# ducha-aiki/affnet

Measured on AMD Instinct MI355X. Metric: keypoints/sec (detect+AffNet+OriNet+HardNet) per image, 2000 kp @1024x768, higher is better.
Workload: dtype f32

## Files before the change

### affnet_amd/_lib.py

```python
import ctypes as C
import os

_HERE = os.path.dirname(os.path.abspath(__file__))
LIB_PATH = os.environ.get("AFFNET_HIP_LIB") or os.path.join(_HERE, "libaffnet_hip.so")
PROBES_LIB_PATH = os.path.join(_HERE, "libaffnet_hip_probes.so")

MAX_OCTAVES, MAX_LEVELS, MAX_TAPS = 16, 8, 37
NET_AFFNET, NET_ORINET, NET_HARDNET, NET_AFFNET_FULLCONV = 0, 1, 2, 3
ARITH_FP32_MFMA, ARITH_FP32_SPLIT3, ARITH_FP32_SPLIT2H = 0, 1, 2
ARITH_NAMES = {"fp32": ARITH_FP32_MFMA, "fp32_mfma": ARITH_FP32_MFMA, "fp32_split3": ARITH_FP32_SPLIT3, "split3": ARITH_FP32_SPLIT3,
               "fp32_split2h": ARITH_FP32_SPLIT2H, "split2h": ARITH_FP32_SPLIT2H}


def arith_code(arith):
    if arith is None:
        return ARITH_FP32_MFMA
    if isinstance(arith, str):
        if arith.lower() not in ARITH_NAMES:
            raise ValueError("arith must be one of %s" % sorted(ARITH_NAMES))
        return ARITH_NAMES[arith.lower()]
    if int(arith) not in (ARITH_FP32_MFMA, ARITH_FP32_SPLIT3, ARITH_FP32_SPLIT2H):
        raise ValueError("arith must be AFFNET_ARITH_FP32_MFMA (0), AFFNET_ARITH_FP32_SPLIT3 (1) or AFFNET_ARITH_FP32_SPLIT2H (2)")
    return int(arith)
SHAPE_FORM_DIRECT, SHAPE_FORM_WINOGRAD = 0, 1
OK, ERR_INVALID, ERR_HIP, ERR_CAPACITY, ERR_EMPTY = 0, -1, -2, -3, -4


class Config(C.Structure):
    _fields_ = [
        ("height", C.c_int32), ("width", C.c_int32), ("n_octaves", C.c_int32), ("levels_per_octave", C.c_int32),
        ("oct_h", C.c_int32 * MAX_OCTAVES), ("oct_w", C.c_int32 * MAX_OCTAVES),
        ("level_sigma", (C.c_float * MAX_LEVELS) * MAX_OCTAVES),
        ("level_sigma4", (C.c_float * MAX_LEVELS) * MAX_OCTAVES),
        ("level_sigma_px", (C.c_double * MAX_LEVELS) * MAX_OCTAVES),
        ("first_blur_taps", C.c_int32), ("first_blur", C.c_float * (MAX_TAPS * MAX_TAPS)),
        ("level_blur_taps", C.c_int32 * MAX_LEVELS),
        ("level_blur", (C.c_float * (MAX_TAPS * MAX_TAPS)) * MAX_LEVELS),
        ("level_blur0_taps", C.c_int32 * MAX_LEVELS),
        ("level_blur0", (C.c_float * (MAX_TAPS * MAX_TAPS)) * MAX_LEVELS),
        ("lazy_shape_rows", C.c_int32),
        ("onepass", C.c_int32),
        ("mr_size", C.c_float), ("threshold", C.c_float),
        ("num_features", C.c_int32), ("num_prefilter", C.c_int32),
        ("max_raw_per_octave_div", C.c_int32), ("max_keep", C.c_int32), ("batch", C.c_int32), ("baum_iters", C.c_int32),
        ("arith", C.c_int32),
    ]


class Nets(C.Structure):
    _fields_ = [("d_affnet", C.c_void_p), ("d_orinet", C.c_void_p), ("d_hardnet", C.c_void_p),
                ("h_orientation_window", C.c_void_p), ("h_baumberg_window", C.c_void_p)]


_P, _I, _SZ = C.c_void_p, C.c_int, C.c_size_t
SYMBOLS = {
    "affnet_config_fill": (_I, [C.POINTER(Config), _I, _I, _I, C.c_double, _I, C.c_double, C.c_double, _I, _I, _I, _I]),
    "affnet_ctx_create": (_I, [C.POINTER(_P), _I, C.POINTER(Config)]),
    "affnet_ctx_destroy": (None, [_P]),
    "affnet_last_error": (C.c_char_p, [_P]),
    "affnet_version": (C.c_char_p, []),
    "affnet_set_arith": (_I, [_P, _I]),
    "affnet_get_arith": (_I, [_P]),
    "affnet_set_shape_form": (_I, [_P, _I]),
    "affnet_get_shape_form": (_I, [_P]),
    "affnet_workspace_bytes": (_SZ, [_P]),
    "affnet_bind_workspace": (_I, [_P, _P, _SZ]),
    "affnet_pyramid_level_offset": (C.c_int64, [_P, _I, _I]),
    "affnet_pyramid_image_stride": (C.c_int64, [_P]),
    "affnet_batch": (_I, [_P]),
    "affnet_capacity_prefilter": (_I, [_P]),
    "affnet_capacity_final": (_I, [_P]),
    "affnet_gauss_blur": (_I, [_P, _P, _P, _I, _I, C.POINTER(C.c_float), _I, _P]),
    "affnet_pyramid_build": (_I, [_P, _P, _P]),
    "affnet_hessian_response": (_I, [_P, _P, _P, _I, _I, C.c_float, _P]),
    "affnet_detect": (_I, [_P, _P, _P, _P, _P, _P]),
    "affnet_detect_responses": (_I, [_P, _P, _P, _P, _P, _P, _P]),
    "affnet_laf_grid_sample": (_I, [_P, _P, _I, _I, _P, _I, _I, _P, _P]),
    "affnet_pyr_grid_sample": (_I, [_P, _P, _P, _P, _I, _I, _P, _P]),
    "affnet_cnn32_packed_floats": (_SZ, [_I]),
    "affnet_cnn32_winograd_offset": (C.c_int64, [_I, _I]),
    "affnet_cnn32_pack_weights": (_I, [_I, C.POINTER(_P), C.POINTER(_P), C.POINTER(_P), _P, _P, _P, _P, _P]),
    "affnet_cnn32_forward": (_I, [_P, _I, _P, _P, _P, _I, _P, _P, _P]),
    "affnet_cnn32_forward_pyr": (_I, [_P, _I, _P, _P, _P, _P, _I, _P, _P, _P]),
    "affnet_local_norm": (_I, [_P, _P, _P, _I, _I, _P]),
    "affnet_fullconv_scratch_bytes": (_SZ, [_I, _I]),
    "affnet_fullconv_forward": (_I, [_P, _P, _P, _I, _I, _P, _P, _P]),
    "affnet_nms2d": (_I, [_P, _P, _P, _I, _I, C.c_float, _P]),
    "affnet_shape_filter_select": (_I, [_P, _P, _P, _P, _P, _P, _P, _P, _P, _P, _P]),
    "affnet_apply_rotation": (_I, [_P, _P, _P, _P, _I, _P]),
    "affnet_scale_lafs": (_I, [_P, _P, _P, _P, _I, _I, _I, _I, _P]),
    "affnet_lafs_to_ellipses": (_I, [_P, _P, _P, _I, _P, _P]),
    "affnet_ellipses_to_lafs": (_I, [_P, _P, _P, _I, _P, _P]),
    "affnet_level_select": (_I, [_P, _P, _P, _I, _I, _P, _P, _P]),
    "affnet_handcrafted_forward": (_I, [_P, _I, _P, _I, _P, _P, _P, _P]),
    "affnet_handcrafted_forward_pyr": (_I, [_P, _I, _P, _P, _P, _I, _P, _P, _P]),
    "affnet_sift_host_window": (_I, [_I, C.POINTER(C.c_float)]),
    "affnet_sift_forward": (_I, [_P, _P, _I, _P, C.c_float, _P, _P]),
    "affnet_sift_forward_pyr": (_I, [_P, _P, _P, _P, _I, _P, C.c_float, _P, _P]),
    "affnet_tfeat_packed_floats": (_SZ, []),
    "affnet_tfeat_pack_weights": (_I, [_P, _P, _P, _P, _P, _P, _P]),
    "affnet_tfeat_scratch_floats": (_SZ, [_I]),
    "affnet_tfeat_forward": (_I, [_P, _P, _P, _P, _I, _P, _P, _P]),
    "affnet_tfeat_forward_pyr": (_I, [_P, _P, _P, _P, _P, _I, _P, _P, _P]),
    "affnet_match_scratch_bytes": (_SZ, [_I, _I]),
    "affnet_distance_matrix": (_I, [_P, _P, _I, _P, _I, _I, _P, _P, _P]),
    "affnet_match_snn": (_I, [_P, _P, _I, _P, _I, _I, C.c_float, _P, _P, _P, _P, _P, _P, _P]),
    "affnet_reproject_lafs": (_I, [_P, _P, _I, C.POINTER(C.c_float), _P, _P]),
    "affnet_centre_nn": (_I, [_P, _P, _I, _P, _I, _P, _P, _P]),
    "affnet_extract_features": (_I, [_P, C.POINTER(Nets), _P, _I, _P, _P, _P, _P, _P, _P]),
    "affnet_detect_image": (_I, [_P, _P, _P]),
    "affnet_detect_image_responses": (_I, [_P, _P, _P]),
    "affnet_detect_image_onepass": (_I, [_P, _P, _P, _P]),
    "affnet_detect_image_onepass_responses": (_I, [_P, _P, _P, _P]),
    "affnet_detected_list": (_I, [_P, _P, _P, _P, _P, _P]),
    "affnet_load_frames": (_I, [_P, _P, _I, _P, _P, _P, _I, _I, _P]),
    "affnet_describe_frames": (_I, [_P, C.POINTER(Nets), _P, _P, _P, _P, _I, _I, _P, _P, _P, _P, _P, _P]),
    "affnet_shape_iterate": (_I, [_P, _P, _P, _P, _P, _I, _P, _P]),
    "affnet_affmap_offset": (C.c_int64, [_P, _I]),
    "affnet_affmap_image_stride": (C.c_int64, [_P]),
    "affnet_describe_detected": (_I, [_P, C.POINTER(Nets), _I, _P, _P, _P, _P, _P, _P]),
    "affnet_graph_capture_extract": (_I, [_P, C.POINTER(Nets), _P, _I, _P, _P, _P, _P, _P, _P]),
    "affnet_graph_launch": (_I, [_P, _P]),
    "affnet_profile_enable": (_I, [_P, _I]),
    "affnet_profile_read": (_I, [_P, C.POINTER(C.c_double * 8), C.POINTER(C.c_int32)]),
    "affnet_read_counts": (_I, [_P, C.POINTER(C.c_int32 * 4), _P]),
    "affnet_counter_offset": (C.c_int64, [_P, _I]),
    "affnet_counter_stride": (C.c_int64, [_P]),
    "affnet_host_base_grid": (_I, [_I, C.POINTER(C.c_float)]),
}

DEBUG_SYMBOLS = {
    "affnet_cnn32_debug_timing": (_I, [_P, _P]),
    "affnet_cnn32_debug_layer": (_I, [_P, _I, _P, _P, _I, _P, _P]),
    "affnet_cnn32_debug_winograd_u": (_I, [_P, _I, _P, _I, _P, _P]),
    "affnet_selftest_mfma": (_I, [_P, _P, _P, _P]),
    "affnet_debug_split3_variant": (_I, [_P, _I]),
}

PROBE_SYMBOLS = {
    "affnet_cnn32_probe": (_I, [_P, _I, _I, _I, _I, _P, _P]),
    "affnet_split3_gemm": (_I, [_P, _P, _I, _I, _I, _I, _P, _P]),
    "affnet_split3_rate": (_I, [_I, _I, _I, _P, _P]),
    "affnet_debug_stream": (_I, [_P, _P, _SZ, _I, _I, _I, _P]),
    "affnet_probe_shape_offsets": (_I, [_P, C.POINTER(C.c_int64 * 3)]),
}


class AffnetHipError(RuntimeError):
    pass


class AffnetEmptyError(AffnetHipError):
    """AFFNET_ERR_EMPTY: no image of the call produced a detection (the reference raises in torch.cat([]),
    SparseImgRepresenter.py:100)."""


def _load():
    if not os.path.isfile(LIB_PATH):
        if os.path.basename(LIB_PATH) == os.path.basename(PROBES_LIB_PATH):
            raise ImportError("affnet_amd: %s is missing - the tools under tools/ need the probe build of the library: "
                              "AFFNET_PROBES=1 bash affnet_amd/csrc/build.sh" % LIB_PATH)
        raise ImportError(
            "affnet_amd: %s is missing - the HIP extension is the only implementation of this path "
            "(no CPU fallback). Build it: bash affnet_amd/csrc/build.sh" % LIB_PATH)
    lib = C.CDLL(LIB_PATH)
    for table in (SYMBOLS, DEBUG_SYMBOLS):
        for name, (res, args) in table.items():
            fn = getattr(lib, name)
            fn.restype, fn.argtypes = res, args
    for name, (res, args) in PROBE_SYMBOLS.items():
        if hasattr(lib, name):
            fn = getattr(lib, name)
            fn.restype, fn.argtypes = res, args
    return lib


lib = _load()


def check(rc, ctx=None, what=""):
    if rc != OK:
        msg = lib.affnet_last_error(ctx).decode() if ctx else ""
        if rc == ERR_EMPTY:
            raise AffnetEmptyError("%s: %s" % (what or "libaffnet_hip call", msg))
        raise AffnetHipError("%s failed (code %d): %s" % (what or "libaffnet_hip call", rc, msg))


def ptr(t):
    return None if t is None else C.c_void_p(t.data_ptr())


def current_stream(device):
    import torch
    return C.c_void_p(torch.cuda.current_stream(device).cuda_stream)
```

### affnet_amd/csrc/cnn_trunk.h

```cpp
#pragma once
#include <math.h>

#include <type_traits>

#include "common.h"

#include "cnn_mfma.h"

template <int TM>
__device__ __forceinline__ void head_partials(const float* __restrict__ hw, const f32x4 (&bias)[1], const f32x4 (&acc)[TM][1],
                                              float* __restrict__ part, int wave, int lane) {
    constexpr int MT = 4, MG = MT / TM;
    const int mg = wave % MG, ng = wave / MG;
    const int n = lane & 15, g = lane >> 4;
    const int c4 = ng * 16 + 4 * g;
    f32x4 v[TM];
#pragma unroll
    for (int i = 0; i < TM; ++i) {
        v[i] = acc[i][0] + bias[0];
        v[i].x = fmaxf(v[i].x, 0.0f); v[i].y = fmaxf(v[i].y, 0.0f); v[i].z = fmaxf(v[i].z, 0.0f); v[i].w = fmaxf(v[i].w, 0.0f);
    }
    const __amdgpu_buffer_rsrc_t r = weight_rsrc(hw, 3 * 4096);
    f32x4 w[3][TM];
#pragma unroll
    for (int o = 0; o < 3; ++o)
#pragma unroll
        for (int i = 0; i < TM; ++i) w[o][i] = buf_read4(r, (n * 64 + c4) * 4, (o * 4096 + (mg * TM + i) * 16 * 64) * 4);
#pragma unroll
    for (int o = 0; o < 3; ++o) {
        float sacc = 0.f;
#pragma unroll
        for (int i = 0; i < TM; ++i)
#pragma unroll
            for (int j = 0; j < 4; ++j) sacc = fmaf(v[i][j], w[o][i][j], sacc);
        sacc = wave_sum(sacc);
        if (lane == 0) part[wave * 4 + o] = sacc;
    }
}

#define ORI_HP 68
struct OriHeadLane {
    int mg, n, c4;
    template <int TM>
    __device__ __forceinline__ static OriHeadLane of(int wave, int lane) {
        constexpr int MT = 4, MG = MT / TM;
        const int mg = wave % MG, ng = wave / MG;
        const int n = lane & 15, g = lane >> 4;
        return {mg, n, ng * 16 + 4 * g};
    }
};
template <int TM>
__device__ __forceinline__ void ori_head_weights(const float* __restrict__ hw, const OriHeadLane& L, f32x4 (&w)[2][TM]) {
    const __amdgpu_buffer_rsrc_t r = weight_rsrc(hw, 2 * 4096);
#pragma unroll
    for (int o = 0; o < 2; ++o)
#pragma unroll
        for (int i = 0; i < TM; ++i) w[o][i] = buf_read4(r, (L.n * 64 + L.c4) * 4, (o * 4096 + (L.mg * TM + i) * 16 * 64) * 4);
}
template <int NTHR>
__device__ __forceinline__ void ori_head_zero_halo(float* act, int tid) {
    for (int e = tid; e < 36 * 16; e += NTHR) {
        const int hp = e >> 4, q4 = e & 15;
        const int y = hp < 10 ? 0 : (hp < 20 ? 9 : 1 + ((hp - 20) >> 1)), x = hp < 10 ? hp : (hp < 20 ? hp - 10 : ((hp - 20) & 1) * 9);
        *reinterpret_cast<f32x4*>(&act[(y * 10 + x) * ORI_HP + 4 * q4]) = (f32x4){0.f, 0.f, 0.f, 0.f};
    }
}
template <int TM>
__device__ __forceinline__ void ori_head_pbase(const OriHeadLane& L, int (&pbase)[TM]) {
#pragma unroll
    for (int i = 0; i < TM; ++i) {
        const int p = (L.mg * TM + i) * 16 + L.n;
        pbase[i] = ((p >> 3) * 10 + (p & 7)) * ORI_HP + L.c4;
    }
}
template <int TM>
__device__ __forceinline__ void ori_head_reduce(const f32x4 (&w)[2][TM], const int (&pbase)[TM], float* __restrict__ part, const float* act, int wave, int lane) {
    __syncthreads();
#pragma unroll
    for (int q = 0; q < 9; ++q) {
        float s0 = 0.f, s1 = 0.f;
#pragma unroll
        for (int i = 0; i < TM; ++i) {
            const f32x4 av = *reinterpret_cast<const f32x4*>(&act[pbase[i] + ((q / 3) * 10 + q % 3) * ORI_HP]);
#pragma unroll
            for (int j = 0; j < 4; ++j) { s0 = fmaf(av[j], w[0][i][j], s0); s1 = fmaf(av[j], w[1][i][j], s1); }
        }
        s0 = wave_sum(s0);
        s1 = wave_sum(s1);
        if (lane == 0) { part[wave * 18 + q] = s0; part[wave * 18 + 9 + q] = s1; }
    }
}
template <int TM, int NTHR>
__device__ __forceinline__ void head_partials_ori_lds(const float* __restrict__ hw, const f32x4 (&bias)[1], const f32x4 (&acc)[TM][1],
                                                      float* __restrict__ part, float* act, int wave, int lane, int tid) {
    constexpr int MT = 4, MG = MT / TM;
    const int mg = wave % MG, ng = wave / MG;
    const int n = lane & 15, g = lane >> 4;
    const int c4 = ng * 16 + 4 * g;
    f32x4 v[TM];
#pragma unroll
    for (int i = 0; i < TM; ++i) {
        v[i] = acc[i][0] + bias[0];
        v[i].x = fmaxf(v[i].x, 0.0f); v[i].y = fmaxf(v[i].y, 0.0f); v[i].z = fmaxf(v[i].z, 0.0f); v[i].w = fmaxf(v[i].w, 0.0f);
    }
    const __amdgpu_buffer_rsrc_t r = weight_rsrc(hw, 2 * 4096);
    f32x4 w[2][TM];
#pragma unroll
    for (int o = 0; o < 2; ++o)
#pragma unroll
        for (int i = 0; i < TM; ++i) w[o][i] = buf_read4(r, (n * 64 + c4) * 4, (o * 4096 + (mg * TM + i) * 16 * 64) * 4);
    __syncthreads();
    for (int e = tid; e < 36 * 16; e += NTHR) {
        const int hp = e >> 4, q4 = e & 15;
        const int y = hp < 10 ? 0 : (hp < 20 ? 9 : 1 + ((hp - 20) >> 1)), x = hp < 10 ? hp : (hp < 20 ? hp - 10 : ((hp - 20) & 1) * 9);
        *reinterpret_cast<f32x4*>(&act[(y * 10 + x) * ORI_HP + 4 * q4]) = (f32x4){0.f, 0.f, 0.f, 0.f};
    }
    int pbase[TM];
#pragma unroll
    for (int i = 0; i < TM; ++i) {
        const int p = (mg * TM + i) * 16 + n;
        pbase[i] = ((p >> 3) * 10 + (p & 7)) * ORI_HP + c4;
        *reinterpret_cast<f32x4*>(&act[pbase[i] + 11 * ORI_HP]) = v[i];
    }
    __syncthreads();
#pragma unroll
    for (int q = 0; q < 9; ++q) {
        float s0 = 0.f, s1 = 0.f;
#pragma unroll
        for (int i = 0; i < TM; ++i) {
            const f32x4 av = *reinterpret_cast<const f32x4*>(&act[pbase[i] + ((q / 3) * 10 + q % 3) * ORI_HP]);
#pragma unroll
            for (int j = 0; j < 4; ++j) { s0 = fmaf(av[j], w[0][i][j], s0); s1 = fmaf(av[j], w[1][i][j], s1); }
        }
        s0 = wave_sum(s0);
        s1 = wave_sum(s1);
        if (lane == 0) { part[wave * 18 + q] = s0; part[wave * 18 + 9 + q] = s1; }
    }
}

#define CNN_STAMP(k)                                                                                     \
    do {                                                                                                 \
        if (STAMPS && a.dbg_time && lane == 0) a.dbg_time[((size_t)pidx * NW + wave) * 32 + (k)] = __builtin_readcyclecounter(); \
    } while (0)

template <int CB>
struct TrunkLds {
    static constexpr int ACT = (CB / 4) * LayC0::PSG;
    static constexpr int PATCH = WP32 * WP32;
    static constexpr int RED = 256;
    static constexpr int TOTAL = ACT + PATCH + RED;
};

template <int KIND, int NW>
struct TrunkShape {
    static constexpr int CB = (KIND == AFFNET_NET_HARDNET) ? 32 : 16;
    static constexpr int NTHR = NW * 64;
    static constexpr int T1M = (CB == 16) ? 8 : 64 / NW, T1N = CB / 16;
    static constexpr int T2M = (CB == 16) ? 4 : 64 / NW, T2N = 1;
    static constexpr int T4M = (CB == 16) ? 2 : 32 / NW, T4N = 1;
    static constexpr int AREG = (NW == 8 && CB == 32) ? 128 : 48;
    static constexpr int G2 = pick_groups(CB, T2M, T2N, 32, AREG), G3 = pick_groups(2 * CB, T2M, T2N, 32, AREG);
    static constexpr int G4 = pick_groups(2 * CB, T4M, T4N, 32, AREG), G5 = pick_groups(4 * CB, T4M, T4N, 32, AREG);
};

template <int C, typename L, int NTHR>
__device__ __forceinline__ void dump_planes(const float* act, float* dst) {
    constexpr int H = L::H;
    for (int i = threadIdx.x; i < C * H * H; i += NTHR) {
        const int c = i / (H * H), r = i - c * H * H, y = r / H, x = r - y * H;
        dst[i] = act[L::at(c, y, x)];
    }
}

template <int CB>
struct SplitLays {
    typedef LayQ<16, 32, 34, CB, 0, 3> LQH;
    typedef LayQ<16, 32, 34, CB, 16, 3> LQH2;
    using LR0 = LayR<32, 32, 34, CB, 0>;
    using LR0H = LayR<16, 32, 34, CB, 0, 34>;
    using LR1 = LayR<32, 32, 34, CB, 16>;
    using LR1H = LayR<16, 32, 34, CB, 16, 34>;
    static_assert(LR0::BYTES <= TrunkLds<CB>::ACT * 4 && LR1::BYTES <= TrunkLds<CB>::ACT * 4 && LR0H::GS == LR0::GS && LR1H::GS == LR1::GS, "whole-patch split layouts");
    static_assert(LQH::BYTES <= TrunkLds<CB>::ACT * 4 && LQH2::BYTES <= TrunkLds<CB>::ACT * 4, "pre-split layouts must fit the activation buffer");
};

template <int KIND, int NW, bool STAMPS, int S3 = 0>
__global__ __launch_bounds__(NW * 64, (KIND == AFFNET_NET_HARDNET) ? NW / 4 : 4) void cnn32_trunk_kernel(CnnArgs a, PyrSrc ps) {
    static_assert(S3 == 0 || S3 == 2 || S3 == 3 || (S3 == 1 && KIND == AFFNET_NET_AFFNET), "S3 = number of terms of the split arithmetic; 1 = exact AffNet with Winograd conv1 / conv3");
    constexpr bool EXACT = S3 <= 1;
    constexpr bool WINO13 = (S3 == 0 && KIND == AFFNET_NET_ORINET) || S3 == 1;
    using S = TrunkShape<KIND, NW>;
    constexpr int CB = S::CB, NTHR = S::NTHR;
    static_assert((CB / 4) * LayC1::PSG <= TrunkLds<CB>::ACT && (CB / 2) * LayC3::PSG <= TrunkLds<CB>::ACT, "LDS layout");
    __shared__ __attribute__((aligned(16))) float lds[TrunkLds<CB>::TOTAL];
    float* act = lds;
    float* patch = lds + TrunkLds<CB>::ACT;
    float* red = patch + TrunkLds<CB>::PATCH;
    const int n = a.count ? min(a.count[blockIdx.y], a.n_max) : a.n_max;
    const int prow = blockIdx.x + a.row_begin;
    if (KIND == AFFNET_NET_AFFNET && a.shape_cnt && blockIdx.x == 0 && threadIdx.x == 0) {
        int32_t* c = a.shape_cnt + (size_t)blockIdx.y * CNT_TOTAL;
        if (a.shape_op == 1) { c[CNT_SURVIVED] = 0; c[CNT_SURVIVED1] = 0; c[CNT_AFF_EVAL] = 0; c[CNT_AFF_REEVAL] = 0; }
        else if (a.shape_op == 2) c[CNT_SURVIVED1] = c[CNT_SURVIVED];
    }
    if (prow >= n || lazy_skip(a.skip_cnt, a.skip_n, blockIdx.y, CNT_SURVIVED)) return;
    const size_t pidx = (size_t)blockIdx.y * a.n_max + prow;
    if (KIND == AFFNET_NET_AFFNET && a.reeval && a.reeval[pidx] == 0) return;
    const int tid = threadIdx.x, wave = tid >> 6, lane = tid & 63;
    if (KIND == AFFNET_NET_HARDNET) __builtin_amdgcn_s_setprio(3);
    CNN_STAMP(0);
    if (STAMPS && a.dbg_time && lane == 0) {
        a.dbg_time[((size_t)pidx * NW + wave) * 32 + 14] = __builtin_amdgcn_s_getreg((31 << 11) | 4);
        a.dbg_time[((size_t)pidx * NW + wave) * 32 + 15] = __builtin_amdgcn_s_getreg((31 << 11) | 20);
    }
    float w0[3][S::T1N];
    f32x4 bias0[S::T1N];
    conv0_load_w<NW, CB, S::T1M, S::T1N>(a.packed + a.off.w[0], a.packed + a.off.b[0], w0, bias0, wave, lane);
    f32x4 b1[1][S::T1N];
    f32x4 Ur[4];
    if constexpr (S3 == 0 && KIND == AFFNET_NET_AFFNET) prefetch_b0<NW, CB, 32, S::T1M, S::T1N, 1>(a.packed + a.off.w[1], b1, wave, lane);
    if constexpr (WINO13) wino_prefetch_u_row<NW, CB, CB, 32, Wino16::NB1>(a.wino_u, Ur, wave, lane);

    constexpr int PPT = 1024 / NTHR;
    constexpr int RPT = 32 / PPT;
    float v[PPT];
    if (a.patches) {
        const float* src = a.patches + pidx * 1024;
#pragma unroll
        for (int q = 0; q < PPT; ++q) v[q] = src[tid + q * NTHR];
    } else {
        int o = a.ids[3 * pidx], l = a.ids[3 * pidx + 1];
        o = o < 0 ? 0 : (o >= ps.t.n_octaves ? ps.t.n_octaves - 1 : o);
        l = l < 0 ? 0 : (l >= ps.t.n_levels ? ps.t.n_levels - 1 : l);
        const float* img = ps.t.lvl[o][l] + blockIdx.y * ps.t.img_stride;
        const int h = ps.t.h[o], w = ps.t.w[o];
        const float* L = a.lafs + 6 * pidx;
        const float m = (float)(h < w ? h : w);
        const float t00 = L[0] * m, t01 = L[1] * m, t02 = L[2] * (float)w;
        const float t10 = L[3] * m, t11 = L[4] * m, t12 = L[5] * (float)h;
#pragma unroll
        for (int q = 0; q < PPT; ++q)
            v[q] = aff_sample_bilinear(img, h, w, t00, t01, t02, t10, t11, t12, ps.base[tid & 31], ps.base[(tid >> 5) + q * RPT]);
    }
    CNN_STAMP(16);
    if (tid < 4 * 33) {
        const int e = tid;
        const int y = e < 34 ? 0 : (e < 68 ? 33 : 1 + ((e - 68) >> 1)), x = e < 34 ? e : (e < 68 ? e - 34 : ((e - 68) & 1) * 33);
        patch[y * WP32 + x] = 0.0f;
    }
    if constexpr (EXACT) zero_halo<LayC0, NTHR>(act, CB);
    else if constexpr (S3 == 2) zero_halo_q<typename SplitLays<CB>::LR0, NTHR>(act);
    else zero_halo_q<typename SplitLays<CB>::LQH, NTHR>(act);
    float sum = 0.f;
#pragma unroll
    for (int q = 0; q < PPT; ++q) sum += v[q];
    const float mean = block_sum<NW>(sum, red) * (1.0f / 1024.0f);
    CNN_STAMP(17);
    float sq = 0.f;
#pragma unroll
    for (int q = 0; q < PPT; ++q) { v[q] -= mean; sq += v[q] * v[q]; }
    const float var = block_sum<NW>(sq, red + NW) * (1.0f / 1023.0f);
    const float sd = sqrtf(var) + 1e-7f;
    CNN_STAMP(18);
#pragma unroll
    for (int q = 0; q < PPT; ++q) patch[((tid >> 5) + q * RPT + 1) * WP32 + (tid & 31) + 1] = v[q] / sd;
    __syncthreads();
    CNN_STAMP(1);

    if constexpr (S3 == 0 && KIND == AFFNET_NET_HARDNET) {
        constexpr int T1M = S::T1M, T1N = S::T1N, T2M = S::T2M, T2N = S::T2N, T4M = S::T4M, T4N = S::T4N;
        constexpr int NB1 = (16 * 16 / 16) * (CB / 16) / NW, NB3 = (8 * 8 / 16) * (2 * CB / 16) / NW, NB5 = (4 * 4 / 16) * (4 * CB / 16) / NW;

        f32x4 Up[2][4];
        f32x4 Uw[16];
        {
            f32x4 acc[T1M][T1N];
            conv0_mfma<NW, CB, T1M, T1N>(patch, w0, bias0, acc, wave, lane);
            CNN_STAMP(19);
            store_tiles_lds<CB, LayC0, T1M, T1N, false>(act, bias0, acc, wave, lane);
            CNN_STAMP(20);
            wino_prefetch_u_pair<NW, CB, CB, 32, NB1>(a.packed + a.off.w_wino[0], Up, wave, lane);
            __syncthreads();
        }
        if (STAMPS && a.dbg_layer == 0) { dump_planes<CB, LayC0, NTHR>(act, a.dbg_out); return; }
        CNN_STAMP(2);

        f32x4 b2[S::G2][T2N];
        f32x4 bias2[T2N];
        {
            f32x4 y[NB1][4], bw[NB1];
            __builtin_amdgcn_s_setprio(0);
            conv3x3_wino_mfma_pair_rows<NW, CB, CB, LayC0, NB1>(act, a.packed + a.off.w_wino[0], Up, y, wave, lane);
            __builtin_amdgcn_s_setprio(3);
            CNN_STAMP(3);
            prefetch_b0<NW, 2 * CB, 16, T2M, T2N, S::G2>(a.packed + a.off.w[2], b2, wave, lane);
            prefetch_bias<NW, 16, T2M, T2N>(a.packed + a.off.b[2], bias2, wave, lane);
            wino_bias<NW, 32, CB, NB1>(a.packed + a.off.b[1], bw, wave, lane);
            __syncthreads();
            CNN_STAMP(21);
            zero_halo<LayC1, NTHR>(act, CB);
            wino_store_lds<CB, LayC1, NB1>(act, bw, y, wave, lane);
            CNN_STAMP(22);
            __syncthreads();
            CNN_STAMP(4);
        }
        if (STAMPS && a.dbg_layer == 1) { dump_planes<CB, LayC1, NTHR>(act, a.dbg_out); return; }

        {
            f32x4 acc[T2M][T2N];
            __builtin_amdgcn_s_setprio(0);
            conv3x3_mfma<NW, CB, 2 * CB, LayC1, 2, T2M, T2N, S::G2>(act, a.packed + a.off.w[2], b2, acc, wave, lane);
            __builtin_amdgcn_s_setprio(3);
            CNN_STAMP(5);
            wino_prefetch_u_pair<NW, 2 * CB, 2 * CB, 16, NB3>(a.packed + a.off.w_wino[1], Up, wave, lane);
            __syncthreads();
            zero_halo<LayC2, NTHR>(act, 2 * CB);
            store_tiles_lds<2 * CB, LayC2, T2M, T2N>(act, bias2, acc, wave, lane);
            __syncthreads();
            CNN_STAMP(6);
        }
        if (STAMPS && a.dbg_layer == 2) { dump_planes<2 * CB, LayC2, NTHR>(act, a.dbg_out); return; }

        f32x4 b4[S::G4][T4N];
        f32x4 bias4[T4N];
        {
            f32x4 y[NB3][4], bw[NB3];
            __builtin_amdgcn_s_setprio(0);
            conv3x3_wino_mfma_pair_rows<NW, 2 * CB, 2 * CB, LayC2, NB3>(act, a.packed + a.off.w_wino[1], Up, y, wave, lane);
            __builtin_amdgcn_s_setprio(3);
            CNN_STAMP(7);
            prefetch_b0<NW, 4 * CB, 8, T4M, T4N, S::G4>(a.packed + a.off.w[4], b4, wave, lane);
            prefetch_bias<NW, 8, T4M, T4N>(a.packed + a.off.b[4], bias4, wave, lane);
            wino_bias<NW, 16, 2 * CB, NB3>(a.packed + a.off.b[3], bw, wave, lane);
            __syncthreads();
            zero_halo<LayC3, NTHR>(act, 2 * CB);
            wino_store_lds<2 * CB, LayC3, NB3>(act, bw, y, wave, lane);
            __syncthreads();
            CNN_STAMP(8);
        }
        if (STAMPS && a.dbg_layer == 3) { dump_planes<2 * CB, LayC3, NTHR>(act, a.dbg_out); return; }

        {
            f32x4 acc[T4M][T4N];
// ... 13 lines not shown
        f32x4 y[NB5][4], bw[NB5];
        __builtin_amdgcn_s_setprio(0);
        static_assert(NB5 == 1 && (4 * CB / 16) * 4096 <= TrunkLds<CB>::ACT, "conv5: one pass per wave, V of the layer fits the activation buffer");
        conv3x3_wino_mfma_shared_v<NW, 4 * CB, 4 * CB, LayC4>(act, a.packed + a.off.w_wino[2], Uw, y, wave, lane);
        __builtin_amdgcn_s_setprio(3);
        CNN_STAMP(11);
        wino_bias<NW, 8, 4 * CB, NB5>(a.packed + a.off.b[5], bw, wave, lane);
        if (!STAMPS || a.dbg_layer < 0) {
            wino_store_global<4 * CB, 8, NB5>(a.out + pidx * (64 * 4 * CB), bw, y, wave, lane);
            CNN_STAMP(13);
            return;
        }
        __syncthreads();
        wino_store_lds<4 * CB, LayC5, NB5>(act, bw, y, wave, lane);
        __syncthreads();
        CNN_STAMP(12);
        if (STAMPS && a.dbg_layer == 5) { dump_planes<4 * CB, LayC5, NTHR>(act, a.dbg_out); return; }
    } else if constexpr (EXACT) {
        constexpr int T1M = S::T1M, T1N = S::T1N, T2M = S::T2M, T2N = S::T2N, T4M = S::T4M, T4N = S::T4N;
        static_assert(NW == 8 && CB == 16, "Wino16 describes the 16-channel trunks on 8 waves");
        f32x4 b4[S::G4][T4N];
        f32x4 bias4[T4N];
        if constexpr (WINO13) {
            constexpr int NB1 = Wino16::NB1, NB3 = Wino16::NB3;
            {
                f32x4 acc[T1M][T1N];
                conv0_mfma<NW, CB, T1M, T1N>(patch, w0, bias0, acc, wave, lane);
                CNN_STAMP(19);
                store_tiles_lds<CB, LayC0, T1M, T1N, false>(act, bias0, acc, wave, lane);
                CNN_STAMP(20);
                __syncthreads();
            }
            if (STAMPS && a.dbg_layer == 0) { dump_planes<CB, LayC0, NTHR>(act, a.dbg_out); return; }
            CNN_STAMP(2);

            f32x4 b2[S::G2][T2N];
            f32x4 bias2[T2N];
            {
                f32x4 y[NB1][4], bw[NB1];
                conv3x3_wino_mfma_rows<NW, CB, CB, LayC0, NB1>(act, a.wino_u, Ur, y, wave, lane);
                CNN_STAMP(3);
                prefetch_b0<NW, 2 * CB, 16, T2M, T2N, S::G2>(a.packed + a.off.w[2], b2, wave, lane);
                prefetch_bias<NW, 16, T2M, T2N>(a.packed + a.off.b[2], bias2, wave, lane);
                wino_bias<NW, 32, CB, NB1>(a.packed + a.off.b[1], bw, wave, lane);
                __syncthreads();
                CNN_STAMP(21);
                zero_halo<LayC1, NTHR>(act, CB);
                wino_store_lds<CB, LayC1, NB1>(act, bw, y, wave, lane);
                CNN_STAMP(22);
                __syncthreads();
                CNN_STAMP(4);
            }
            if (STAMPS && a.dbg_layer == 1) { dump_planes<CB, LayC1, NTHR>(act, a.dbg_out); return; }

            {
                f32x4 acc[T2M][T2N];
                conv3x3_mfma<NW, CB, 2 * CB, LayC1, 2, T2M, T2N, S::G2>(act, a.packed + a.off.w[2], b2, acc, wave, lane);
                CNN_STAMP(5);
                wino_prefetch_u_row<NW, 2 * CB, 2 * CB, 16, NB3>(a.wino_u + Wino16::offset(3), Ur, wave, lane);
                __syncthreads();
                zero_halo<LayC2, NTHR>(act, 2 * CB);
                store_tiles_lds<2 * CB, LayC2, T2M, T2N>(act, bias2, acc, wave, lane);
                __syncthreads();
                CNN_STAMP(6);
            }
            if (STAMPS && a.dbg_layer == 2) { dump_planes<2 * CB, LayC2, NTHR>(act, a.dbg_out); return; }

            {
                f32x4 y[NB3][4], bw[NB3];
                conv3x3_wino_mfma_rows<NW, 2 * CB, 2 * CB, LayC2, NB3>(act, a.wino_u + Wino16::offset(3), Ur, y, wave, lane);
                CNN_STAMP(7);
                prefetch_b0<NW, 4 * CB, 8, T4M, T4N, S::G4>(a.packed + a.off.w[4], b4, wave, lane);
                prefetch_bias<NW, 8, T4M, T4N>(a.packed + a.off.b[4], bias4, wave, lane);
                wino_bias<NW, 16, 2 * CB, NB3>(a.packed + a.off.b[3], bw, wave, lane);
                __syncthreads();
                zero_halo<LayC3, NTHR>(act, 2 * CB);
                wino_store_lds<2 * CB, LayC3, NB3>(act, bw, y, wave, lane);
                __syncthreads();
                CNN_STAMP(8);
            }
            if (STAMPS && a.dbg_layer == 3) { dump_planes<2 * CB, LayC3, NTHR>(act, a.dbg_out); return; }

        } else {
            static_assert(T1M * 8 > S::AREG, "conv1: two A sets of T1M float4 do not fit -> rolling single set (conv3x3_mfma_roll)");
            f32x4 bias1[T1N];
            {
                f32x4 acc[T1M][T1N];
                conv0_mfma<NW, CB, T1M, T1N>(patch, w0, bias0, acc, wave, lane);
                CNN_STAMP(19);
                prefetch_bias<NW, 32, T1M, T1N>(a.packed + a.off.b[1], bias1, wave, lane);
                store_tiles_lds<CB, LayC0, T1M, T1N, false>(act, bias0, acc, wave, lane);
                CNN_STAMP(20);
                __syncthreads();
            }
            if (STAMPS && a.dbg_layer == 0) { dump_planes<CB, LayC0, NTHR>(act, a.dbg_out); return; }
            CNN_STAMP(2);

            f32x4 b2[S::G2][T2N];
            f32x4 bias2[T2N];
            {
                f32x4 acc[T1M][T1N];
                conv3x3_mfma_roll<NW, CB, CB, LayC0, 1, T1M, T1N>(act, a.packed + a.off.w[1], b1, acc, wave, lane);
                CNN_STAMP(3);
                prefetch_b0<NW, 2 * CB, 16, T2M, T2N, S::G2>(a.packed + a.off.w[2], b2, wave, lane);
                prefetch_bias<NW, 16, T2M, T2N>(a.packed + a.off.b[2], bias2, wave, lane);
                __syncthreads();
                CNN_STAMP(21);
                zero_halo<LayC1, NTHR>(act, CB);
                store_tiles_lds<CB, LayC1, T1M, T1N>(act, bias1, acc, wave, lane);
                CNN_STAMP(22);
                __syncthreads();
                CNN_STAMP(4);
            }
            if (STAMPS && a.dbg_layer == 1) { dump_planes<CB, LayC1, NTHR>(act, a.dbg_out); return; }

            f32x4 b3[S::G3][T2N];
            f32x4 bias3[T2N];
            {
                f32x4 acc[T2M][T2N];
                conv3x3_mfma<NW, CB, 2 * CB, LayC1, 2, T2M, T2N, S::G2>(act, a.packed + a.off.w[2], b2, acc, wave, lane);
                CNN_STAMP(5);
                prefetch_b0<NW, 2 * CB, 16, T2M, T2N, S::G3>(a.packed + a.off.w[3], b3, wave, lane);
                prefetch_bias<NW, 16, T2M, T2N>(a.packed + a.off.b[3], bias3, wave, lane);
                __syncthreads();
                zero_halo<LayC2, NTHR>(act, 2 * CB);
                store_tiles_lds<2 * CB, LayC2, T2M, T2N>(act, bias2, acc, wave, lane);
                __syncthreads();
                CNN_STAMP(6);
            }
            if (STAMPS && a.dbg_layer == 2) { dump_planes<2 * CB, LayC2, NTHR>(act, a.dbg_out); return; }

            {
                f32x4 acc[T2M][T2N];
                conv3x3_mfma<NW, 2 * CB, 2 * CB, LayC2, 1, T2M, T2N, S::G3>(act, a.packed + a.off.w[3], b3, acc, wave, lane);
                CNN_STAMP(7);
                prefetch_b0<NW, 4 * CB, 8, T4M, T4N, S::G4>(a.packed + a.off.w[4], b4, wave, lane);
                prefetch_bias<NW, 8, T4M, T4N>(a.packed + a.off.b[4], bias4, wave, lane);
                __syncthreads();
                zero_halo<LayC3, NTHR>(act, 2 * CB);
                store_tiles_lds<2 * CB, LayC3, T2M, T2N>(act, bias3, acc, wave, lane);
                __syncthreads();
                CNN_STAMP(8);
            }
            if (STAMPS && a.dbg_layer == 3) { dump_planes<2 * CB, LayC3, NTHR>(act, a.dbg_out); return; }

        }

        f32x4 b5[S::G5][T4N];
        f32x4 bias5[T4N];
        {
            f32x4 acc[T4M][T4N];
            conv3x3_mfma<NW, 2 * CB, 4 * CB, LayC3, 2, T4M, T4N, S::G4>(act, a.packed + a.off.w[4], b4, acc, wave, lane);
            CNN_STAMP(9);
            if constexpr (KIND == AFFNET_NET_ORINET) {
                wino5_prefetch_u(a.wino_u + Wino16::offset(5), Ur, wave, lane);
            } else {
                prefetch_b0<NW, 4 * CB, 8, T4M, T4N, S::G5>(a.packed + a.off.w[5], b5, wave, lane);
                prefetch_bias<NW, 8, T4M, T4N>(a.packed + a.off.b[5], bias5, wave, lane);
            }
            __syncthreads();
            zero_halo<LayC4, NTHR>(act, 4 * CB);
            store_tiles_lds<4 * CB, LayC4, T4M, T4N>(act, bias4, acc, wave, lane);
            __syncthreads();
            CNN_STAMP(10);
        }
        if (STAMPS && a.dbg_layer == 4) { dump_planes<4 * CB, LayC4, NTHR>(act, a.dbg_out); return; }

        if constexpr (KIND == AFFNET_NET_ORINET) {
            static_assert(Wino5::X >= 16 * LayC4::PSG && Wino5::X + Wino5::X_FLOATS <= TrunkLds<CB>::TOTAL && Wino5::HEAD + 100 * ORI_HP <= Wino5::X,
                          "conv5: the exchange lies behind conv4's output inside the LDS array, the head copy in front of the exchange");
            f32x4 acc[2][4], y[2], hw[2][T4M];
            conv3x3_wino_mfma_half_rows<NW, LayC4>(act, a.wino_u + Wino16::offset(5), Ur, acc, wave, lane);
            CNN_STAMP(11);
            const f32x4 bw = *reinterpret_cast<const f32x4*>(&a.packed[a.off.b[5] + (wave >> 1) * 16 + 4 * (lane >> 4)]);
            const OriHeadLane HL = OriHeadLane::of<T4M>(wave, lane);
            if (!STAMPS || a.dbg_layer < 0) ori_head_weights<T4M>(a.packed + a.off.head_w, HL, hw);
            wino5_combine(lds, acc, y, wave, lane);
            if (!STAMPS || a.dbg_layer < 0) {
                float* copy = lds + Wino5::HEAD;
                ori_head_zero_halo<NTHR>(copy, tid);
                wino5_store_lds<10, ORI_HP, 4>(copy + 11 * ORI_HP, bw, y, wave, lane);
                int pbase[T4M];
                ori_head_pbase<T4M>(HL, pbase);
                ori_head_reduce<T4M>(hw, pbase, a.out + pidx * HEAD_PART_ORI, copy, wave, lane);
                CNN_STAMP(13);
                return;
            }
            __syncthreads();
            wino5_store_lds<LayC5::WP, 4, LayC5::PSG>(act + (LayC5::WP + 1) * 4, bw, y, wave, lane);
            __syncthreads();
            CNN_STAMP(12);
            if (STAMPS && a.dbg_layer == 5) { dump_planes<4 * CB, LayC5, NTHR>(act, a.dbg_out); return; }
            return;
        }
        f32x4 acc[T4M][T4N];
        conv3x3_mfma<NW, 4 * CB, 4 * CB, LayC4, 1, T4M, T4N, S::G5>(act, a.packed + a.off.w[5], b5, acc, wave, lane);
        CNN_STAMP(11);
        if (!STAMPS || a.dbg_layer < 0) {
            head_partials<T4M>(a.packed + a.off.head_w, bias5, acc, a.out + pidx * HEAD_PART_AFF, wave, lane);
            CNN_STAMP(13);
            return;
        }
        __syncthreads();
        store_tiles_lds<4 * CB, LayC5, T4M, T4N>(act, bias5, acc, wave, lane);
        __syncthreads();
        CNN_STAMP(12);
        if (STAMPS && a.dbg_layer == 5) { dump_planes<4 * CB, LayC5, NTHR>(act, a.dbg_out); return; }
    } else if constexpr (KIND == AFFNET_NET_HARDNET) {
        using SL = SplitLays<CB>;
        using LQH = typename SL::LQH;
        using LQH2 = typename SL::LQH2;
        using LR0 = typename SL::LR0;
        using LR1 = typename SL::LR1;
        constexpr int TERMS = S3;
        constexpr bool WHOLE = TERMS == 2;
        f32x4 bias1[2];
        const int s3_alt = a.s3_alt;
        using LQ2 = std::conditional_t<TERMS == 2, LayR<16, 16, 20, 2 * CB, 16>, LayQ<16, 16, 18, 2 * CB, 0, 3>>;
        using LQ4 = std::conditional_t<TERMS == 2, LayR<8, 8, 12, 4 * CB, 0>, LayQ<8, 8, 16, 4 * CB, 128, 3>>;
        static_assert(LQ2::BYTES <= TrunkLds<CB>::ACT * 4 && LQ4::BYTES <= TrunkLds<CB>::ACT * 4, "pre-split layouts must fit the activation buffer");
        char* base = reinterpret_cast<char*>(act);
        f32x4 acc_a[4][2], acc_b[4][2];
        S3W<2> wf1;
        S3W<1> wf2;
        f32x4 acc2_a[4][1], acc2_b[4][1], bias2[1];
        f32x4 acc2w[4][2], bias2w[2];
        if constexpr (WHOLE) {
            f32x4 acc1[8][2];
            S3W<2> wf2w;
            s3_prefetch_w0<NW, CB, CB, 64, 8, 2, TERMS>(a.packed + a.off.w_s3[1], wf1, wave, lane);
            prefetch_bias<NW, 32, 8, 2>(a.packed + a.off.b[1], bias1, wave, lane);
            conv0_whole_split_q<NW, LR0, 2>(patch, w0, bias0, act, wave, lane);
            __syncthreads();
            CNN_STAMP(2);
            __builtin_amdgcn_s_setprio(0);
            conv3x3_mfma_s3q<NW, CB, CB, LR0, 1, 8, 2>(act, a.packed + a.off.w_s3[1], wf1, acc1, wave, lane, s3_alt);
            __builtin_amdgcn_s_setprio(3);
            CNN_STAMP(3);
            s3_prefetch_w0<NW, CB, 2 * CB, 16, 4, 2, TERMS>(a.packed + a.off.w_s3[2], wf2w, wave, lane);
            prefetch_bias<NW, 16, 4, 2>(a.packed + a.off.b[2], bias2w, wave, lane);
            __syncthreads();
            zero_halo_q<LR1, NTHR>(act);
            store_tiles_split_q<CB, LR1, 8, 2>(act, bias1, acc1, wave, lane);
            __syncthreads();
            CNN_STAMP(4);
            __builtin_amdgcn_s_setprio(0);
            conv3x3_mfma_s3q<NW, CB, 2 * CB, LR1, 2, 4, 2>(act, a.packed + a.off.w_s3[2], wf2w, acc2w, wave, lane, s3_alt);
            __builtin_amdgcn_s_setprio(3);
        } else {
            s3_prefetch_w0<NW, CB, CB, 32, 4, 2, TERMS>(a.packed + a.off.w_s3[1], wf1, wave, lane);
            prefetch_bias<NW, 32, 8, 2>(a.packed + a.off.b[1], bias1, wave, lane);
            conv0_half_split_q<NW, LQH, 2>(patch, w0, bias0, act, 0, wave, lane);
            __syncthreads();
            CNN_STAMP(2);
            __builtin_amdgcn_s_setprio(0);
            conv3x3_mfma_s3q<NW, CB, CB, LQH, 1, 4, 2>(act, a.packed + a.off.w_s3[1], wf1, acc_a, wave, lane, s3_alt);
            __builtin_amdgcn_s_setprio(3);
            __syncthreads();
            if (tid < LQH::SLOTS * 4 * 32) {
                const int t = tid / 128, g = (tid >> 5) & 3, x = tid & 31;
                *reinterpret_cast<f32x4*>(base + g * LQH::GS + LQH::at(17, x + 1) + t * LQH::TSTEP) = (f32x4){0.f, 0.f, 0.f, 0.f};
            }
            conv0_half_split_q<NW, LQH, 2>(patch, w0, bias0, act, 1, wave, lane);
            __syncthreads();
            __builtin_amdgcn_s_setprio(0);
            conv3x3_mfma_s3q<NW, CB, CB, LQH, 1, 4, 2>(act, a.packed + a.off.w_s3[1], wf1, acc_b, wave, lane, s3_alt);
            __builtin_amdgcn_s_setprio(3);
            CNN_STAMP(3);
            s3_prefetch_w0<NW, CB, 2 * CB, 8, 4, 1, TERMS>(a.packed + a.off.w_s3[2], wf2, wave, lane);
            bias2[0] = *reinterpret_cast<const f32x4*>(&a.packed[a.off.b[2] + (wave >> 1) * 16 + 4 * (lane >> 4)]);
            __syncthreads();
            zero_halo_q<LQH2, NTHR>(act);
            store_tiles_split_q<CB, LQH2, 4, 2>(act, bias1, acc_a, wave, lane);
            __syncthreads();
            CNN_STAMP(4);
            __builtin_amdgcn_s_setprio(0);
            conv3x3_mfma_s3q<NW, CB, 2 * CB, LQH2, 2, 4, 1>(act, a.packed + a.off.w_s3[2], wf2, acc2_a, wave, lane, s3_alt);
            __builtin_amdgcn_s_setprio(3);
            __syncthreads();
            store_tiles_split_q<CB, LQH2, 4, 2>(act, bias1, acc_b, wave, lane);
            if (wave == 7) {
                const int n = lane & 15;
#pragma unroll
                for (int i = 2; i < 4; ++i) split_store_tile_q<LQH2, 2>(base, LQH2::at(0, (i - 2) * 16 + n + 1), 0, bias1, acc_a[i], lane >> 4);
            }
            __syncthreads();
            __builtin_amdgcn_s_setprio(0);
            conv3x3_mfma_s3q<NW, CB, 2 * CB, LQH2, 2, 4, 1>(act, a.packed + a.off.w_s3[2], wf2, acc2_b, wave, lane, s3_alt);
            __builtin_amdgcn_s_setprio(3);
        }
        CNN_STAMP(5);
        S3W<2> wf3;
        S3W<1> wf4, wf5;
        f32x4 bias3[2], bias4[1], bias5s[1];
        s3_prefetch_w0<NW, 2 * CB, 2 * CB, 16, 4, 2, TERMS>(a.packed + a.off.w_s3[3], wf3, wave, lane);
        prefetch_bias<NW, 16, 4, 2>(a.packed + a.off.b[3], bias3, wave, lane);
        __syncthreads();
        zero_halo_q<LQ2, NTHR>(act);
        if constexpr (WHOLE) store_tiles_split_q<2 * CB, LQ2, 4, 2>(act, bias2w, acc2w, wave, lane);
        else {
            store_tiles_split_q<2 * CB, LQ2, 4, 1, 8>(act, bias2, acc2_a, wave, lane, 0);
            store_tiles_split_q<2 * CB, LQ2, 4, 1, 8>(act, bias2, acc2_b, wave, lane, 8);
        }
        __syncthreads();
        CNN_STAMP(6);
        {
            f32x4 acc_[4][2];
            __builtin_amdgcn_s_setprio(0);
            conv3x3_mfma_s3q<NW, 2 * CB, 2 * CB, LQ2, 1, 4, 2>(act, a.packed + a.off.w_s3[3], wf3, acc_, wave, lane, s3_alt);
            __builtin_amdgcn_s_setprio(3);
            CNN_STAMP(7);
            s3_prefetch_w0<NW, 2 * CB, 4 * CB, 4, 4, 1, TERMS>(a.packed + a.off.w_s3[4], wf4, wave, lane);
            prefetch_bias<NW, 8, 4, 1>(a.packed + a.off.b[4], bias4, wave, lane);
            __syncthreads();
            store_tiles_split_q<2 * CB, LQ2, 4, 2>(act, bias3, acc_, wave, lane);
            __syncthreads();
            CNN_STAMP(8);
        }
        {
            f32x4 acc_[4][1];
            __builtin_amdgcn_s_setprio(0);
            conv3x3_mfma_s3q<NW, 2 * CB, 4 * CB, LQ2, 2, 4, 1>(act, a.packed + a.off.w_s3[4], wf4, acc_, wave, lane, s3_alt);
            __builtin_amdgcn_s_setprio(3);
            CNN_STAMP(9);
            s3_prefetch_w0<NW, 4 * CB, 4 * CB, 4, 4, 1, TERMS>(a.packed + a.off.w_s3[5], wf5, wave, lane);
            prefetch_bias<NW, 8, 4, 1>(a.packed + a.off.b[5], bias5s, wave, lane);
            __syncthreads();
            zero_halo_q<LQ4, NTHR>(act);
            store_tiles_split_q<4 * CB, LQ4, 4, 1>(act, bias4, acc_, wave, lane);
            __syncthreads();
            CNN_STAMP(10);
        }
        f32x4 acc5[4][1];
        __builtin_amdgcn_s_setprio(0);
        conv3x3_mfma_s3q<NW, 4 * CB, 4 * CB, LQ4, 1, 4, 1>(act, a.packed + a.off.w_s3[5], wf5, acc5, wave, lane, s3_alt);
        __builtin_amdgcn_s_setprio(3);
        CNN_STAMP(11);
// ... 132 lines not shown
```

### affnet_amd/csrc/debug.hip

```cpp
#include "common.h"

#include "../../include/affnet_hip_probes.h"

template <typename T>
__global__ __launch_bounds__(256) void stream_read_kernel(const T* __restrict__ src, float* __restrict__ dst, size_t n_items) {
    float acc = 0.f;
    for (size_t i = (size_t)blockIdx.x * 256 + threadIdx.x; i < n_items; i += (size_t)gridDim.x * 256) {
        const T v = src[i];
        const float* f = reinterpret_cast<const float*>(&v);
#pragma unroll
        for (int k = 0; k < (int)(sizeof(T) / 4); ++k) acc += f[k];
    }
    if (acc == 123.456f) dst[blockIdx.x] = acc;
    if (threadIdx.x == 0 && blockIdx.x == 0) dst[0] = acc;
}

template <typename T>
__global__ __launch_bounds__(256) void stream_write_kernel(T* __restrict__ dst, size_t n_items) {
    T v;
    float* f = reinterpret_cast<float*>(&v);
#pragma unroll
    for (int k = 0; k < (int)(sizeof(T) / 4); ++k) f[k] = (float)(threadIdx.x + k);
    for (size_t i = (size_t)blockIdx.x * 256 + threadIdx.x; i < n_items; i += (size_t)gridDim.x * 256) dst[i] = v;
}

__global__ __launch_bounds__(256) void tile_read_kernel(const float* __restrict__ img, float* __restrict__ dst, int h, int w, int halo) {
    const int LW = 64 + 2 * halo, n_el = LW * LW;
    const int x0 = blockIdx.x * 64, y0 = blockIdx.y * 64;
    float acc = 0.f;
    for (int i = threadIdx.x; i < n_el; i += 256) {
        const int ty = i / LW, tx = i - ty * LW;
        int gy = y0 + ty - halo, gx = x0 + tx - halo;
        gy = gy < 0 ? 0 : (gy >= h ? h - 1 : gy);
        gx = gx < 0 ? 0 : (gx >= w ? w - 1 : gx);
        acc += img[(size_t)gy * w + gx];
    }
    if (acc == 123.456f) dst[blockIdx.x] = acc;
}

struct f32x2s { float a, b; };

extern "C" int affnet_debug_stream(const void* d_src, void* d_dst, size_t n_bytes, int width, int mode, int halo, void* stream) {
    if (!d_dst || n_bytes == 0 || (n_bytes & 65535) != 0) return AFFNET_ERR_INVALID;
    hipStream_t st = (hipStream_t)stream;
    const int blocks = 256 * 16;
    if (mode == 0) {
        if (!d_src) return AFFNET_ERR_INVALID;
        if (width == 4) hipLaunchKernelGGL(stream_read_kernel<float>, dim3(blocks), dim3(256), 0, st, (const float*)d_src, (float*)d_dst, n_bytes / 4);
        else if (width == 8) hipLaunchKernelGGL(stream_read_kernel<f32x2s>, dim3(blocks), dim3(256), 0, st, (const f32x2s*)d_src, (float*)d_dst, n_bytes / 8);
        else if (width == 16) hipLaunchKernelGGL(stream_read_kernel<float4>, dim3(blocks), dim3(256), 0, st, (const float4*)d_src, (float*)d_dst, n_bytes / 16);
        else return AFFNET_ERR_INVALID;
    } else if (mode == 1) {
        if (width == 4) hipLaunchKernelGGL(stream_write_kernel<float>, dim3(blocks), dim3(256), 0, st, (float*)d_dst, n_bytes / 4);
        else if (width == 8) hipLaunchKernelGGL(stream_write_kernel<f32x2s>, dim3(blocks), dim3(256), 0, st, (f32x2s*)d_dst, n_bytes / 8);
        else if (width == 16) hipLaunchKernelGGL(stream_write_kernel<float4>, dim3(blocks), dim3(256), 0, st, (float4*)d_dst, n_bytes / 16);
        else return AFFNET_ERR_INVALID;
    } else if (mode == 2) {
        if (!d_src || halo < 0 || halo > 16) return AFFNET_ERR_INVALID;
        const int w = 4096, h = (int)(n_bytes / 4 / w);
        hipLaunchKernelGGL(tile_read_kernel, dim3(w / 64, (h + 63) / 64), dim3(256), 0, st, (const float*)d_src, (float*)d_dst, h, w, halo);
    } else {
        return AFFNET_ERR_INVALID;
    }
    return hipGetLastError() == hipSuccess ? AFFNET_OK : AFFNET_ERR_HIP;
}

extern "C" int affnet_probe_shape_offsets(const affnet_ctx* ctx, int64_t out[3]) {
    if (!ctx || !ctx->ws || !out) return AFFNET_ERR_INVALID;
    out[0] = (int64_t)(reinterpret_cast<const char*>(ctx->st_A) - ctx->ws) / 4;
    out[1] = (int64_t)(reinterpret_cast<const char*>(ctx->st_hard_scratch) - ctx->ws) / 4 + (int64_t)ctx->B * ctx->cap_pre * HEAD_PART_AFF;
    out[2] = (int64_t)(reinterpret_cast<const char*>(ctx->st_det_lafs) - ctx->ws) / 4;
    return AFFNET_OK;
}
```

### include/affnet_hip_probes.h

```cpp
#ifndef AFFNET_HIP_PROBES_H
#define AFFNET_HIP_PROBES_H

#include "affnet_hip.h"

#ifdef __cplusplus
extern "C" {
#endif

int affnet_cnn32_probe(const float* d_packed, int layer, int probe, int reps, int n_blocks, float* d_out, void* stream);

int affnet_debug_stream(const void* d_src, void* d_dst, size_t n_bytes, int width, int mode, int halo, void* stream);

int affnet_split3_gemm(const float* d_A, const float* d_Bt, int M, int N, int K, int mode, float* d_C, void* stream);
int affnet_split3_rate(int reps, int terms, int n_blocks, float* d_out, void* stream);

int affnet_probe_shape_offsets(const affnet_ctx* ctx, int64_t out[3]);

#ifdef __cplusplus
}
#endif
#endif
```

Measured before the change: 1.514 million.

## Add Winograd conv5 with fused head to exact AffNet trunk and probes

Extends the Winograd conv5 path, previously used only by OriNet, to the exact-arithmetic AffNet trunk variant. It adds a head-weight loader and partial-sum routine matched to the Winograd output lane mapping, so the affine head reduces directly from conv5 registers. It also adds probe entry points to run the Winograd AffNet kernel per layer and on patch batches. This is meant to cut conv5 multiply work, at the cost of extra transform work and LDS exchange, and possible numerical differences.

After: 1.557 million (median of 6 runs). +2.8%, better.

```diff
diff --git a/affnet_amd/_lib.py b/affnet_amd/_lib.py
--- a/affnet_amd/_lib.py
+++ b/affnet_amd/_lib.py
@@ -143,6 +143,8 @@
     "affnet_split3_rate": (_I, [_I, _I, _I, _P, _P]),
     "affnet_debug_stream": (_I, [_P, _P, _SZ, _I, _I, _I, _P]),
     "affnet_probe_shape_offsets": (_I, [_P, C.POINTER(C.c_int64 * 3)]),
+    "affnet_probe_affnet_wino_layer": (_I, [_P, _I, _P, _P, _I, _P, _P]),
+    "affnet_probe_affnet_wino_partials": (_I, [_P, _P, _P, _I, _P, _P]),
 }
 
 
diff --git a/affnet_amd/csrc/cnn_trunk.h b/affnet_amd/csrc/cnn_trunk.h
--- a/affnet_amd/csrc/cnn_trunk.h
+++ b/affnet_amd/csrc/cnn_trunk.h
@@ -33,6 +33,31 @@
         for (int i = 0; i < TM; ++i)
 #pragma unroll
             for (int j = 0; j < 4; ++j) sacc = fmaf(v[i][j], w[o][i][j], sacc);
+        sacc = wave_sum(sacc);
+        if (lane == 0) part[wave * 4 + o] = sacc;
+    }
+}
+
+__device__ __forceinline__ void aff_head_weights_wino(const float* __restrict__ hw, f32x4 (&w)[3][2], int wave, int lane) {
+    const __amdgpu_buffer_rsrc_t r = weight_rsrc(hw, 3 * 4096);
+    const int m = lane & 15, c4 = (wave >> 1) * 16 + 4 * (lane >> 4);
+    const int pix = (2 * (m >> 2) + (wave & 1)) * 8 + 2 * (m & 3);
+#pragma unroll
+    for (int o = 0; o < 3; ++o)
+#pragma unroll
+        for (int k = 0; k < 2; ++k) w[o][k] = buf_read4(r, (pix * 64 + c4) * 4, (o * 4096 + k * 64) * 4);
+}
+__device__ __forceinline__ void head_partials_wino(const f32x4 (&w)[3][2], f32x4 bias, const f32x4 (&y)[2], float* __restrict__ part, int wave, int lane) {
+    f32x4 v[2];
+#pragma unroll
+    for (int k = 0; k < 2; ++k) v[k] = bias_relu(y[k], bias);
+#pragma unroll
+    for (int o = 0; o < 3; ++o) {
+        float sacc = 0.f;
+#pragma unroll
+        for (int k = 0; k < 2; ++k)
+#pragma unroll
+            for (int j = 0; j < 4; ++j) sacc = fmaf(v[k][j], w[o][k][j], sacc);
         sacc = wave_sum(sacc);
         if (lane == 0) part[wave * 4 + o] = sacc;
     }
@@ -186,9 +211,10 @@
 
 template <int KIND, int NW, bool STAMPS, int S3 = 0>
 __global__ __launch_bounds__(NW * 64, (KIND == AFFNET_NET_HARDNET) ? NW / 4 : 4) void cnn32_trunk_kernel(CnnArgs a, PyrSrc ps) {
-    static_assert(S3 == 0 || S3 == 2 || S3 == 3 || (S3 == 1 && KIND == AFFNET_NET_AFFNET), "S3 = number of terms of the split arithmetic; 1 = exact AffNet with Winograd conv1 / conv3");
+    static_assert(S3 == 0 || S3 == 2 || S3 == 3 || (S3 == 1 && KIND == AFFNET_NET_AFFNET), "S3 = number of terms of the split arithmetic; 1 = exact AffNet with Winograd conv1 / conv3 / conv5");
     constexpr bool EXACT = S3 <= 1;
     constexpr bool WINO13 = (S3 == 0 && KIND == AFFNET_NET_ORINET) || S3 == 1;
+    constexpr bool WINO5 = (S3 == 0 && KIND == AFFNET_NET_ORINET) || S3 == 1;
     using S = TrunkShape<KIND, NW>;
     constexpr int CB = S::CB, NTHR = S::NTHR;
     static_assert((CB / 4) * LayC1::PSG <= TrunkLds<CB>::ACT && (CB / 2) * LayC3::PSG <= TrunkLds<CB>::ACT, "LDS layout");
@@ -508,7 +534,7 @@
             f32x4 acc[T4M][T4N];
             conv3x3_mfma<NW, 2 * CB, 4 * CB, LayC3, 2, T4M, T4N, S::G4>(act, a.packed + a.off.w[4], b4, acc, wave, lane);
             CNN_STAMP(9);
-            if constexpr (KIND == AFFNET_NET_ORINET) {
+            if constexpr (WINO5) {
                 wino5_prefetch_u(a.wino_u + Wino16::offset(5), Ur, wave, lane);
             } else {
                 prefetch_b0<NW, 4 * CB, 8, T4M, T4N, S::G5>(a.packed + a.off.w[5], b5, wave, lane);
@@ -522,9 +548,10 @@
         }
         if (STAMPS && a.dbg_layer == 4) { dump_planes<4 * CB, LayC4, NTHR>(act, a.dbg_out); return; }
 
+        static_assert(!WINO5 || (Wino5::X >= 16 * LayC4::PSG && Wino5::X + Wino5::X_FLOATS <= TrunkLds<CB>::TOTAL),
+                      "Winograd conv5: the exchange lies behind conv4's output inside the LDS array");
         if constexpr (KIND == AFFNET_NET_ORINET) {
-            static_assert(Wino5::X >= 16 * LayC4::PSG && Wino5::X + Wino5::X_FLOATS <= TrunkLds<CB>::TOTAL && Wino5::HEAD + 100 * ORI_HP <= Wino5::X,
-                          "conv5: the exchange lies behind conv4's output inside the LDS array, the head copy in front of the exchange");
+            static_assert(Wino5::HEAD + 100 * ORI_HP <= Wino5::X, "conv5: the head copy in front of the exchange");
             f32x4 acc[2][4], y[2], hw[2][T4M];
             conv3x3_wino_mfma_half_rows<NW, LayC4>(act, a.wino_u + Wino16::offset(5), Ur, acc, wave, lane);
             CNN_STAMP(11);
@@ -539,6 +566,24 @@
                 int pbase[T4M];
                 ori_head_pbase<T4M>(HL, pbase);
                 ori_head_reduce<T4M>(hw, pbase, a.out + pidx * HEAD_PART_ORI, copy, wave, lane);
+                CNN_STAMP(13);
+                return;
+            }
+            __syncthreads();
+            wino5_store_lds<LayC5::WP, 4, LayC5::PSG>(act + (LayC5::WP + 1) * 4, bw, y, wave, lane);
+            __syncthreads();
+            CNN_STAMP(12);
+            if (STAMPS && a.dbg_layer == 5) { dump_planes<4 * CB, LayC5, NTHR>(act, a.dbg_out); return; }
+            return;
+        } else if constexpr (WINO5) {
+            f32x4 acc[2][4], y[2], hw[3][2];
+            conv3x3_wino_mfma_half_rows<NW, LayC4>(act, a.wino_u + Wino16::offset(5), Ur, acc, wave, lane);
+            CNN_STAMP(11);
+            const f32x4 bw = *reinterpret_cast<const f32x4*>(&a.packed[a.off.b[5] + (wave >> 1) * 16 + 4 * (lane >> 4)]);
+            if (!STAMPS || a.dbg_layer < 0) aff_head_weights_wino(a.packed + a.off.head_w, hw, wave, lane);
+            wino5_combine(lds, acc, y, wave, lane);
+            if (!STAMPS || a.dbg_layer < 0) {
+                head_partials_wino(hw, bw, y, a.out + pidx * HEAD_PART_AFF, wave, lane);
                 CNN_STAMP(13);
                 return;
             }
diff --git a/affnet_amd/csrc/debug.hip b/affnet_amd/csrc/debug.hip
--- a/affnet_amd/csrc/debug.hip
+++ b/affnet_amd/csrc/debug.hip
@@ -72,3 +72,32 @@
     out[2] = (int64_t)(reinterpret_cast<const char*>(ctx->st_det_lafs) - ctx->ws) / 4;
     return AFFNET_OK;
 }
+
+static int probe_affnet_wino(affnet_ctx* ctx, const float* d_packed, const float* d_patches, int n, float* d_out, int layer, hipStream_t st) {
+    if (ctx->arith != AFFNET_ARITH_FP32_MFMA) return aff_fail(ctx, AFFNET_ERR_INVALID, "probe_affnet_wino: AFFNET_ARITH_FP32_MFMA only");
+    const NetLayout L = net_layout(AFFNET_NET_AFFNET);
+    CnnArgs a;
+    memset(&a, 0, sizeof(a));
+    a.packed = d_packed; a.off = to_offsets(L, ctx->arith);
+    const int rc = aff_wino_derive_u(ctx, AFFNET_NET_AFFNET, d_packed, L, st, &a.wino_u);
+    if (rc) return rc;
+    a.patches = d_patches; a.n_max = n; a.out = d_out; a.dbg_layer = layer; a.dbg_out = d_out; a.dbg_time = ctx->dbg_time;
+    PyrSrc ps;
+    memset(&ps, 0, sizeof(ps));
+    hipLaunchKernelGGL(aff_trunk_affnet_wino(layer >= 0 || a.dbg_time), dim3(n, 1), dim3(512), 0, st, a, ps);
+    AFF_LAUNCH_CHECK(ctx);
+    return AFFNET_OK;
+}
+
+extern "C" int affnet_probe_affnet_wino_layer(affnet_ctx* ctx, int net_kind, const float* d_packed, const float* d_patch, int layer, float* d_out, void* stream) {
+    AFF_DEVICE(ctx);
+    if (!ctx || !d_packed || !d_patch || !d_out || net_kind != AFFNET_NET_AFFNET || layer < 0 || layer > 5)
+        return aff_fail(ctx, AFFNET_ERR_INVALID, "probe_affnet_wino_layer: AffNet, layer 0 .. 5");
+    return probe_affnet_wino(ctx, d_packed, d_patch, 1, d_out, layer, (hipStream_t)stream);
+}
+
+extern "C" int affnet_probe_affnet_wino_partials(affnet_ctx* ctx, const float* d_packed, const float* d_patches, int n, float* d_partials, void* stream) {
+    AFF_DEVICE(ctx);
+    if (!ctx || !d_packed || !d_patches || !d_partials || n < 1 || n > 65535) return aff_fail(ctx, AFFNET_ERR_INVALID, "probe_affnet_wino_partials: bad argument");
+    return probe_affnet_wino(ctx, d_packed, d_patches, n, d_partials, -1, (hipStream_t)stream);
+}
diff --git a/include/affnet_hip_probes.h b/include/affnet_hip_probes.h
--- a/include/affnet_hip_probes.h
+++ b/include/affnet_hip_probes.h
@@ -16,6 +16,10 @@
 
 int affnet_probe_shape_offsets(const affnet_ctx* ctx, int64_t out[3]);
 
+int affnet_probe_affnet_wino_layer(affnet_ctx* ctx, int net_kind, const float* d_packed, const float* d_patch, int layer, float* d_out, void* stream);
+
+int affnet_probe_affnet_wino_partials(affnet_ctx* ctx, const float* d_packed, const float* d_patches, int n, float* d_partials, void* stream);
+
 #ifdef __cplusplus
 }
 #endif
```
